# lucidrains/audiolm-pytorch

Hardware: NVIDIA H100
Metric: CoarseTransformer tokens/sec fwd+bwd seq2048 (higher is better)
Workload: dtype bf16

## Files before the change

audiolm_pytorch_b200/csrc/attn_bwd_wgmma.cu:

```cuda
#include "alm_common.cuh"
#include "ptx_sm90.cuh"

namespace alm {

constexpr int AB_T = 128;
constexpr int AB_THREADS = 256;
constexpr int AB_STAGES = 3;
template <int D>
struct AttBwdCfg {
  static constexpr int TQ = D == 128 ? 64 : 128;
  static constexpr int ROW_BYTES = SwizzledTile<D>::ROW_BYTES;
  static constexpr int KV_HALF = AB_T * ROW_BYTES, KV_TILE = AB_T * D * 2;
  static constexpr int Q_HALF = TQ * ROW_BYTES, Q_TILE = TQ * D * 2;
  static constexpr int DS_HALF = AB_T * 128, DS_TILE = AB_T * TQ * 2;
  static constexpr int DQ_STAGE = D == 128 ? 2 * 64 * 64 * 4 : 0;
  static constexpr int SMEM = 2 * KV_TILE + 2 * AB_STAGES * Q_TILE + 2 * DS_TILE + DQ_STAGE + AB_STAGES * 2 * TQ * 4 + 256;
};
constexpr float LOG2E = 1.4426950408889634f;

struct AttnBwdParams {
  const float* lse;
  const float* delta;
  const uint32_t* kmask;
  int kb_stride;
  const float* bias;
  float* dbias;
  long long bias_hs, bias_rs;
  float* dq_acc;
  __nv_bfloat16* dk;
  __nv_bfloat16* dv;
  long long lddk, lddv;
  int b, h, n_q, n_k, n_q_pad;
  int causal;
  float scale, scale_log2;
};

__device__ __forceinline__ float ex2_approx(float x) {
  float y;
  asm("ex2.approx.ftz.f32 %0, %1;" : "=f"(y) : "f"(x));
  return y;
}

template <int KS>
__device__ __forceinline__ void pack_a_frags(const float (&v)[8 * KS], uint32_t (&a)[KS][4]) {
#pragma unroll
  for (int kk = 0; kk < KS; ++kk) {
    a[kk][0] = pack_bf16x2(v[8 * kk + 0], v[8 * kk + 1]);
    a[kk][1] = pack_bf16x2(v[8 * kk + 2], v[8 * kk + 3]);
    a[kk][2] = pack_bf16x2(v[8 * kk + 4], v[8 * kk + 5]);
    a[kk][3] = pack_bf16x2(v[8 * kk + 6], v[8 * kk + 7]);
  }
}

template <int D>
__device__ __forceinline__ void store_acc(const float (&acc)[D / 2], __nv_bfloat16* row0, __nv_bfloat16* row1, int c_lane) {
#pragma unroll
  for (int h = 0; h < 2; ++h) {
    __nv_bfloat16* dst = h == 0 ? row0 : row1;
    if (dst == nullptr) continue;
#pragma unroll
    for (int g = 0; g < D / 8; ++g)
      *reinterpret_cast<uint32_t*>(dst + 8 * g + c_lane) = pack_bf16x2(acc[4 * g + 2 * h], acc[4 * g + 2 * h + 1]);
  }
}

template <int TQ>
__device__ __forceinline__ uint64_t attn_bwd_keep_bits(const DropoutArgs& d, uint32_t qrow0, uint32_t key0) {
  uint64_t bits = 0;
#pragma unroll
  for (int cc = 0; cc < TQ / 16; ++cc) {
    const uint32_t i0 = qrow0 + 16 * cc;
    const uint4 dr = dropout_draw(d, i0, key0);
#pragma unroll
    for (int gh = 0; gh < 2; ++gh)
#pragma unroll
      for (int h = 0; h < 2; ++h)
#pragma unroll
        for (int c = 0; c < 2; ++c)
          if (dropout_pick(d, dr, i0 + 8 * gh + c, key0 + 8 * h)) bits |= 1ull << (8 * cc + 4 * gh + 2 * h + c);
  }
  return bits;
}

constexpr uint32_t AB_DS_BAR = 1;
constexpr uint32_t AB_WG_BAR = 2;

constexpr int AB_TRACE_ITERS = 128, AB_TRACE_STAMPS = 8;
#ifdef ALM_ATTN_BWD_TRACE
__device__ long long g_attn_bwd_trace[2][AB_TRACE_ITERS][AB_TRACE_STAMPS];
#define AB_STAMP(i)                                                                                   \
  do {                                                                                                \
    if (blockIdx.x == 0 && (threadIdx.x & 127) == 0 && it < AB_TRACE_ITERS)                           \
      g_attn_bwd_trace[threadIdx.x >> 7][it][i] = clock64();                                          \
  } while (0)
#else
#define AB_STAMP(i)
#endif

template <int AB_D, bool HAS_BIAS, bool DROPOUT>
__global__ void __launch_bounds__(AB_THREADS, 1)
mqa_attn_bwd_kernel(const __grid_constant__ CUtensorMap tmQ, const __grid_constant__ CUtensorMap tmK,
                    const __grid_constant__ CUtensorMap tmV, const __grid_constant__ CUtensorMap tmdO,
                    const __grid_constant__ CUtensorMap tmdQ, const AttnBwdParams p, const DropoutArgs drop) {
  extern __shared__ __align__(1024) uint8_t smem[];
  if ((smem_u32(smem) & 1023u) != 0) __trap();
  using Tile = SwizzledTile<AB_D>;
  using Cfg = AttBwdCfg<AB_D>;
  constexpr int TQ = Cfg::TQ, AB_TILE = Cfg::Q_TILE, AB_DS_TILE = Cfg::DS_TILE;
  constexpr int KV_HALF = Cfg::KV_HALF, Q_HALF = Cfg::Q_HALF, DS_HALF = Cfg::DS_HALF;
  constexpr int WG_ROWS = 64 * Cfg::ROW_BYTES;
  uint8_t* sK = smem;
  uint8_t* sV = sK + Cfg::KV_TILE;
  uint8_t* sQ = sV + Cfg::KV_TILE;
  uint8_t* sdO = sQ + AB_STAGES * AB_TILE;
  uint8_t* sDS = sdO + AB_STAGES * AB_TILE;
  uint8_t* sDQ = sDS + 2 * AB_DS_TILE;
  float* sLse = reinterpret_cast<float*>(sDQ + Cfg::DQ_STAGE);
  float* sDelta = sLse + AB_STAGES * TQ;
  uint64_t* bars = reinterpret_cast<uint64_t*>(sDelta + AB_STAGES * TQ);
  uint64_t* kv_full = bars;
  uint64_t* qdo_full = bars + 1;
  uint64_t* qdo_empty = qdo_full + AB_STAGES;

  const int warp = threadIdx.x >> 5, lane = threadIdx.x & 31;
  const int kb = blockIdx.x / p.b, batch = blockIdx.x % p.b;
  const int k0 = kb * AB_T;
  const int off = p.n_k - p.n_q;
  const int n_qblocks = (p.n_q + TQ - 1) / TQ;
  int qb_min = 0;
  if (p.causal && k0 - off > 0) qb_min = (k0 - off) / TQ;
  const int q_per_head = n_qblocks - qb_min;
  const int n_iter = q_per_head > 0 ? q_per_head * p.h : 0;

  if (threadIdx.x == 0) {
    tma_prefetch_desc(&tmQ); tma_prefetch_desc(&tmK); tma_prefetch_desc(&tmV); tma_prefetch_desc(&tmdO);
    tma_prefetch_desc(&tmdQ);
    mbar_init(kv_full, 1);
    for (int i = 0; i < AB_STAGES; ++i) { mbar_init(&qdo_full[i], 1); mbar_init(&qdo_empty[i], 8); }
    fence_mbar_init();
  }
  __syncthreads();

  auto issue_qdo = [&](int it) {
    const int st = it % AB_STAGES;
    const int head = it / q_per_head, qb = qb_min + it % q_per_head;
    const size_t roff = ((size_t)batch * p.h + head) * p.n_q_pad + (size_t)qb * TQ;
    if (elect_one_sync()) {
      mbar_arrive_expect_tx(&qdo_full[st], 2 * AB_TILE + 2 * TQ * 4);
#pragma unroll
      for (int hf = 0; hf < Tile::HALVES; ++hf) {
        tma_load_3d(sQ + st * AB_TILE + hf * Q_HALF, &tmQ, &qdo_full[st], head * AB_D + hf * Tile::HW, qb * TQ, batch);
        tma_load_3d(sdO + st * AB_TILE + hf * Q_HALF, &tmdO, &qdo_full[st], head * AB_D + hf * Tile::HW, qb * TQ, batch);
      }
      bulk_copy_g2s(sLse + st * TQ, p.lse + roff, TQ * 4, &qdo_full[st]);
      bulk_copy_g2s(sDelta + st * TQ, p.delta + roff, TQ * 4, &qdo_full[st]);
    }
    __syncwarp();
  };
  if (warp == 0 && n_iter > 0) {
    if (elect_one_sync()) {
      mbar_arrive_expect_tx(kv_full, 2 * Cfg::KV_TILE);
#pragma unroll
      for (int hf = 0; hf < Tile::HALVES; ++hf) {
        tma_load_3d(sK + hf * KV_HALF, &tmK, kv_full, hf * Tile::HW, k0, batch);
        tma_load_3d(sV + hf * KV_HALF, &tmV, kv_full, hf * Tile::HW, k0, batch);
      }
    }
    __syncwarp();
    for (int it = 0; it < min(n_iter, AB_STAGES); ++it) issue_qdo(it);
  }

  const int cw = warp >> 2;
  const int wl = warp & 3;
  const int r_base = cw * 64 + wl * 16 + (lane >> 2);
  const int c_lane = 2 * (lane & 3);
  int kj[2];
  bool key_ok[2];
#pragma unroll
  for (int h = 0; h < 2; ++h) {
    kj[h] = k0 + r_base + 8 * h;
    key_ok[h] = kj[h] < p.n_k;
    if (key_ok[h] && p.kmask != nullptr)
      key_ok[h] = (p.kmask[(size_t)batch * p.kb_stride + (kj[h] >> 5)] >> (kj[h] & 31)) & 1u;
  }
  float dv[AB_D / 2], dk[AB_D / 2];
#pragma unroll
  for (int e = 0; e < AB_D / 2; ++e) { dv[e] = 0.f; dk[e] = 0.f; }
  const uint32_t k_all = smem_u32(sK);
  const uint32_t k_addr = k_all + cw * WG_ROWS, v_addr = smem_u32(sV) + cw * WG_ROWS;
  const bool wg_leader = (threadIdx.x & 127) == 0;
  if (n_iter > 0) mbar_wait(kv_full, 0);
  int stage = 0;
  uint32_t phase = 0;
  for (int it = 0; it < n_iter; ++it) {
    const int head = it / q_per_head;
    const int q0 = (qb_min + it % q_per_head) * TQ;
    [[maybe_unused]] const long long bias_head = HAS_BIAS ? (long long)head * p.bias_hs : 0;
    AB_STAMP(0);
    mbar_wait(&qdo_full[stage], phase);
    AB_STAMP(1);
    const uint32_t q_addr = smem_u32(sQ + stage * AB_TILE), do_addr = smem_u32(sdO + stage * AB_TILE);
    const uint32_t ds_addr = smem_u32(sDS + (it & 1) * AB_DS_TILE);
    float st[TQ / 2], dpt[TQ / 2];
    wgmma_fence();
#pragma unroll
    for (int k = 0; k < AB_D / 16; ++k)
      wgmma_ss<TQ>(st, Tile::kmajor(k_addr, k, KV_HALF), Tile::kmajor(q_addr, k, Q_HALF), k > 0 ? 1u : 0u);
    wgmma_commit();
#pragma unroll
    for (int k = 0; k < AB_D / 16; ++k)
      wgmma_ss<TQ>(dpt, Tile::kmajor(v_addr, k, KV_HALF), Tile::kmajor(do_addr, k, Q_HALF), k > 0 ? 1u : 0u);
    wgmma_commit();
    AB_STAMP(2);
    [[maybe_unused]] uint64_t keep = 0;
    if constexpr (DROPOUT)
      keep = attn_bwd_keep_bits<TQ>(drop, ((uint32_t)batch * p.h + head) * (uint32_t)p.n_q_pad + q0 + c_lane, kj[0]);
    const float* lse_s = sLse + stage * TQ;
    const float* del_s = sDelta + stage * TQ;
    const bool tile_full = (q0 + TQ <= p.n_q) && (!p.causal || k0 + AB_T - 1 <= q0 + off);
    const int q_end = tile_full ? INT_MAX : p.n_q;
    int q_lo[2];
#pragma unroll
    for (int h = 0; h < 2; ++h) q_lo[h] = tile_full || !p.causal ? INT_MIN : kj[h] - off;
    auto visible = [&](int h, int qi) { return key_ok[h] & (qi >= q_lo[h]) & (qi < q_end); };
    auto bias_index = [&](int h, int qi) {
      return bias_head + (long long)min(qi, p.n_q - 1) * p.bias_rs + min(kj[h], p.n_k - 1);
    };
    wgmma_wait<1>();
    wgmma_fence_acc(st);
#pragma unroll
    for (int g = 0; g < TQ / 8; ++g)
#pragma unroll
      for (int c = 0; c < 2; ++c) {
        const int col = 8 * g + c_lane + c;
        const int qi = q0 + col;
        const float lv = lse_s[col];
#pragma unroll
        for (int h = 0; h < 2; ++h) {
          const int e = 4 * g + 2 * h + c;
          float shift = -lv;
          if constexpr (HAS_BIAS) shift = fmaf(__ldg(p.bias + bias_index(h, qi)), LOG2E, shift);
          const float x = fmaf(st[e], p.scale_log2, shift);
          st[e] = ex2_approx(visible(h, qi) ? x : -INFINITY);
        }
      }
    AB_STAMP(3);
    uint32_t pa[TQ / 16][4];
    if constexpr (DROPOUT) {
      float pz[TQ / 2];
#pragma unroll
      for (int e = 0; e < TQ / 2; ++e) pz[e] = ((keep >> e) & 1u) ? st[e] * drop.scale : 0.f;
      pack_a_frags(pz, pa);
    } else {
      pack_a_frags(st, pa);
    }
    wgmma_fence_acc(dv);
    wgmma_fence();
#pragma unroll
    for (int kk = 0; kk < TQ / 16; ++kk)
      wgmma_rs<AB_D, 1>(dv, pa[kk], Tile::mnmajor(do_addr, kk, Q_HALF), 1u);
    wgmma_commit();
    wgmma_wait<1>();
    wgmma_fence_acc(dpt);
    if (it > 0) {
      if (wg_leader) bulk_wait_group_read<0>();
      named_bar_sync(AB_WG_BAR + cw, 128);
    }
#pragma unroll
    for (int g = 0; g < TQ / 8; ++g) {
#pragma unroll
      for (int c = 0; c < 2; ++c) {
        const int col = 8 * g + c_lane + c;
        const int qi = q0 + col;
        const float dl = del_s[col];
#pragma unroll
        for (int h = 0; h < 2; ++h) {
          const int e = 4 * g + 2 * h + c;
          const bool ok = visible(h, qi);
          float ds;
          if constexpr (DROPOUT)
            ds = ok ? st[e] * ((((keep >> e) & 1u) ? dpt[e] * drop.scale : 0.f) - dl) : 0.f;
          else
            ds = ok ? st[e] * (dpt[e] - dl) : 0.f;
          if constexpr (HAS_BIAS) {
            if (ok && p.dbias != nullptr) atomicAdd(p.dbias + bias_index(h, qi), ds);
          }
          dpt[e] = ds * p.scale;
        }
      }
#pragma unroll
      for (int h = 0; h < 2; ++h) {
        const int row = r_base + 8 * h;
        const uint32_t a = ds_addr + (g >> 3) * DS_HALF + row * 128 + (((g & 7) ^ (row & 7)) << 4) + 2 * c_lane;
        st_shared_u32(a, pack_bf16x2(dpt[4 * g + 2 * h], dpt[4 * g + 2 * h + 1]));
      }
    }
    AB_STAMP(4);
    fence_proxy_async_smem();
    named_bar_sync(AB_DS_BAR, 2 * 128);
    AB_STAMP(5);
    if (warp == 0 && it >= 1 && it - 1 + AB_STAGES < n_iter) {
      const int prev = stage == 0 ? AB_STAGES - 1 : stage - 1;
      mbar_wait(&qdo_empty[prev], stage == 0 ? phase ^ 1u : phase);
      issue_qdo(it - 1 + AB_STAGES);
    }
    constexpr int DQ_N = AB_D == 128 ? 64 : AB_D;
    float dq[DQ_N / 2];
    wgmma_fence_acc(dk);
    wgmma_fence();
#pragma unroll
    for (int kk = 0; kk < TQ / 16; ++kk)
      wgmma_ss<AB_D, 0, 1>(dk, wgmma_desc_sw128(ds_addr + (kk >> 2) * DS_HALF + cw * 8192 + (kk & 3) * 32, 1024, 16),
                           Tile::mnmajor(q_addr, kk, Q_HALF), 1u);
    const uint32_t dq_a = ds_addr + (AB_D == 128 ? 0 : cw * DS_HALF);
    const uint32_t dq_b = k_all + (AB_D == 128 ? cw * KV_HALF : 0);
#pragma unroll
    for (int kk = 0; kk < AB_T / 16; ++kk)
      wgmma_ss<DQ_N, 1, 1>(dq, wgmma_desc_sw128(dq_a + kk * 2048, 1024, 8192), Tile::mnmajor(dq_b, kk, KV_HALF),
                           kk > 0 ? 1u : 0u);
    wgmma_commit();
    wgmma_wait<0>();
    wgmma_fence_acc(dv);
    wgmma_fence_acc(dk);
    wgmma_fence_acc(dq);
    AB_STAMP(6);
    if (lane == 0) mbar_arrive(&qdo_empty[stage]);
    const uint32_t stg = AB_D == 128 ? smem_u32(sDQ) + cw * (Cfg::DQ_STAGE / 2)
                                     : smem_u32(sDS + ((it + 1) & 1) * AB_DS_TILE) + cw * 8192;
    constexpr uint32_t BOX_STRIDE = AB_D == 128 ? 8192 : DS_HALF;
#pragma unroll
    for (int h = 0; h < 2; ++h) {
      const int row = wl * 16 + (lane >> 2) + 8 * h;
#pragma unroll
      for (int g = 0; g < DQ_N / 8; ++g) {
        const int byte = 32 * (g & 3) + 4 * c_lane;
        st_shared_f32x2(stg + (g >> 2) * BOX_STRIDE + row * 128 + ((((byte >> 4) ^ (row & 7)) << 4) | (byte & 15)),
                        dq[4 * g + 2 * h], dq[4 * g + 2 * h + 1]);
      }
    }
    fence_proxy_async_smem();
    named_bar_sync(AB_WG_BAR + cw, 128);
    if (wg_leader) {
      const int dq_col = head * AB_D + (AB_D == 128 ? cw * 64 : 0), dq_row = q0 + (AB_D == 128 ? 0 : cw * 64);
      tma_reduce_add_3d(&tmdQ, stg, dq_col, dq_row, batch);
      if constexpr (DQ_N == 64) tma_reduce_add_3d(&tmdQ, stg + BOX_STRIDE, dq_col + 32, dq_row, batch);
      bulk_commit_group();
    }
    AB_STAMP(7);
    if (++stage == AB_STAGES) { stage = 0; phase ^= 1u; }
  }
  if (wg_leader) bulk_wait_group<0>();
  __nv_bfloat16* rv[2];
  __nv_bfloat16* rk[2];
#pragma unroll
  for (int h = 0; h < 2; ++h) {
    const bool in = kj[h] < p.n_k;
    rv[h] = in ? p.dv + ((size_t)batch * p.n_k + kj[h]) * p.lddv : nullptr;
    rk[h] = in ? p.dk + ((size_t)batch * p.n_k + kj[h]) * p.lddk : nullptr;
  }
  store_acc<AB_D>(dv, rv[0], rv[1], c_lane);
  store_acc<AB_D>(dk, rk[0], rk[1], c_lane);
}

__global__ void attn_dq_convert_kernel(const float4* __restrict__ acc, __nv_bfloat16* __restrict__ dq, long long lddq,
                                       long long rows, int cols4) {
  const long long i = (long long)blockIdx.x * blockDim.x + threadIdx.x;
  if (i >= rows * cols4) return;
  const long long r = i / cols4;
  const int c = (int)(i - r * cols4);
  const float4 v = acc[i];
  *reinterpret_cast<uint2*>(dq + r * lddq + 4 * c) = make_uint2(pack_bf16x2(v.x, v.y), pack_bf16x2(v.z, v.w));
}

}

namespace alm {
template <int D>
static int attn_bwd_launch(const void* q, int64_t ldq, const void* k, int64_t ldk, int64_t k_bstride, const void* v,
                           int64_t ldv, int64_t v_bstride, const void* d_o, int64_t lddo, void* dq, int64_t lddq,
                           const AttnBwdParams& p, const DropoutArgs& dargs, cudaStream_t stream) {
  using Tile = SwizzledTile<D>;
  using Cfg = AttBwdCfg<D>;
  const int b = p.b, h = p.h, n_q = p.n_q, n_k = p.n_k;
  CUtensorMap tmQ, tmK, tmV, tmdO;
  {
    uint64_t dims[3] = {(uint64_t)h * D, (uint64_t)n_q, (uint64_t)b};
    uint64_t strides[3] = {2, (uint64_t)ldq * 2, (uint64_t)n_q * ldq * 2};
    uint32_t box[3] = {Tile::HW, Cfg::TQ, 1};
    int rc = make_tensor_map(&tmQ, q, 2, 3, dims, strides, box, Tile::SWIZZLE);
    if (rc != ALM_OK) return rc;
    strides[1] = (uint64_t)lddo * 2;
    strides[2] = (uint64_t)n_q * lddo * 2;
    rc = make_tensor_map(&tmdO, d_o, 2, 3, dims, strides, box, Tile::SWIZZLE);
    if (rc != ALM_OK) return rc;
  }
  {
    uint64_t dims[3] = {(uint64_t)D, (uint64_t)n_k, (uint64_t)b};
    uint64_t strides[3] = {2, (uint64_t)ldk * 2, (uint64_t)k_bstride * 2};
    uint32_t box[3] = {Tile::HW, AB_T, 1};
    int rc = make_tensor_map(&tmK, k, 2, 3, dims, strides, box, Tile::SWIZZLE);
    if (rc != ALM_OK) return rc;
    strides[1] = (uint64_t)ldv * 2;
    strides[2] = (uint64_t)v_bstride * 2;
    rc = make_tensor_map(&tmV, v, 2, 3, dims, strides, box, Tile::SWIZZLE);
    if (rc != ALM_OK) return rc;
  }
  CUtensorMap tmdQ;
  {
    uint64_t dims[3] = {(uint64_t)h * D, (uint64_t)n_q, (uint64_t)b};
    uint64_t strides[3] = {4, (uint64_t)h * D * 4, (uint64_t)n_q * h * D * 4};
    uint32_t box[3] = {32, 64, 1};
    int rc = make_tensor_map(&tmdQ, p.dq_acc, 4, 3, dims, strides, box, 128);
    if (rc != ALM_OK) return rc;
  }
  static bool attr_set = false;
  if (!attr_set) {
    ALM_CUDA_OK(cudaFuncSetAttribute(mqa_attn_bwd_kernel<D, false, false>, cudaFuncAttributeMaxDynamicSharedMemorySize, Cfg::SMEM));
    ALM_CUDA_OK(cudaFuncSetAttribute(mqa_attn_bwd_kernel<D, true, false>, cudaFuncAttributeMaxDynamicSharedMemorySize, Cfg::SMEM));
    ALM_CUDA_OK(cudaFuncSetAttribute(mqa_attn_bwd_kernel<D, false, true>, cudaFuncAttributeMaxDynamicSharedMemorySize, Cfg::SMEM));
    ALM_CUDA_OK(cudaFuncSetAttribute(mqa_attn_bwd_kernel<D, true, true>, cudaFuncAttributeMaxDynamicSharedMemorySize, Cfg::SMEM));
    attr_set = true;
  }
  dim3 grid(((n_k + AB_T - 1) / AB_T) * b);
  const bool drop = dargs.thr < 65536u;
  if (p.bias != nullptr && drop)
    mqa_attn_bwd_kernel<D, true, true><<<grid, AB_THREADS, Cfg::SMEM, stream>>>(tmQ, tmK, tmV, tmdO, tmdQ, p, dargs);
  else if (p.bias != nullptr)
    mqa_attn_bwd_kernel<D, true, false><<<grid, AB_THREADS, Cfg::SMEM, stream>>>(tmQ, tmK, tmV, tmdO, tmdQ, p, dargs);
  else if (drop)
    mqa_attn_bwd_kernel<D, false, true><<<grid, AB_THREADS, Cfg::SMEM, stream>>>(tmQ, tmK, tmV, tmdO, tmdQ, p, dargs);
  else
    mqa_attn_bwd_kernel<D, false, false><<<grid, AB_THREADS, Cfg::SMEM, stream>>>(tmQ, tmK, tmV, tmdO, tmdQ, p, dargs);
  ALM_CHECK_LAUNCH();
  const long long rows = (long long)b * n_q;
  const int cols4 = h * D / 4;
  attn_dq_convert_kernel<<<(unsigned)ceil_div(rows * cols4, 256LL), 256, 0, stream>>>(
      reinterpret_cast<const float4*>(p.dq_acc), (__nv_bfloat16*)dq, lddq, rows, cols4);
  ALM_CHECK_LAUNCH();
  ALM_LAUNCHED(2);
  return ALM_OK;
}
}

extern "C" int alm_mqa_attn_bwd_dh(const void* q, int64_t ldq, const void* k, int64_t ldk, int64_t k_bstride,
                                   const void* v, int64_t ldv, int64_t v_bstride, const void* d_o, int64_t lddo,
                                   const void* key_mask, const float* lse, const float* delta, int n_q_pad, void* dq,
                                   int64_t lddq, float* dq_acc, void* dk, int64_t lddk, void* dv, int64_t lddv,
                                   const float* bias, float* dbias, int64_t bias_hstride, int64_t bias_rstride, int b,
                                   int h, int n_q, int n_k, int causal, float scale, float dropout_p, uint64_t seed,
                                   uint32_t site, int dim_head, alm_stream_t stream_) {
  using namespace alm;
  cudaStream_t stream = reinterpret_cast<cudaStream_t>(stream_);
  ALM_REQUIRE(dim_head == 32 || dim_head == 64 || dim_head == 128, ALM_ERR_UNSUPPORTED);
  ALM_REQUIRE(q && k && v && d_o && lse && delta && dq && dq_acc && dk && dv, ALM_ERR_ARG);
  ALM_REQUIRE(b > 0 && h > 0 && n_q > 0 && n_k >= n_q, ALM_ERR_ARG);
  ALM_REQUIRE(n_q_pad % AB_T == 0 && n_q_pad >= n_q, ALM_ERR_ARG);
  ALM_REQUIRE(dropout_p >= 0.f && dropout_p < 1.f, ALM_ERR_ARG);
  ALM_REQUIRE(dropout_p == 0.f || n_q_pad == (n_q + AB_T - 1) / AB_T * AB_T, ALM_ERR_ARG);
  ALM_REQUIRE((long long)b * h * n_q_pad < (1ll << 32), ALM_ERR_UNSUPPORTED);
  if (bias != nullptr) {
    ALM_REQUIRE(bias_rstride >= n_k && bias_rstride % 4 == 0 && bias_hstride % 4 == 0, ALM_ERR_ALIGN);
    ALM_REQUIRE((reinterpret_cast<uintptr_t>(bias) & 15u) == 0, ALM_ERR_ALIGN);
  } else {
    ALM_REQUIRE(dbias == nullptr, ALM_ERR_ARG);
  }
  ALM_REQUIRE(ldq % 8 == 0 && ldk % 8 == 0 && ldv % 8 == 0 && lddo % 8 == 0 && lddq % 8 == 0 && lddk % 8 == 0 &&
                  lddv % 8 == 0 && k_bstride % 8 == 0 && v_bstride % 8 == 0,
              ALM_ERR_ALIGN);
  AttnBwdParams p;
  p.lse = lse; p.delta = delta;
  p.kmask = reinterpret_cast<const uint32_t*>(key_mask);
  p.kb_stride = (n_k + 127) / 128 * 4;
  p.dq_acc = dq_acc; p.dk = (__nv_bfloat16*)dk; p.dv = (__nv_bfloat16*)dv;
  p.lddk = lddk; p.lddv = lddv;
  p.bias = bias; p.dbias = dbias; p.bias_hs = bias_hstride; p.bias_rs = bias_rstride;
  p.b = b; p.h = h; p.n_q = n_q; p.n_k = n_k; p.n_q_pad = n_q_pad;
  p.causal = causal;
  p.scale = scale;
  p.scale_log2 = scale * LOG2E;
  const DropoutArgs dargs = make_dropout_args(dropout_p, seed, site);
#define ALM_ATT_BWD(DD) \
  attn_bwd_launch<DD>(q, ldq, k, ldk, k_bstride, v, ldv, v_bstride, d_o, lddo, dq, lddq, p, dargs, stream)
  if (dim_head == 32) return ALM_ATT_BWD(32);
  if (dim_head == 64) return ALM_ATT_BWD(64);
  return ALM_ATT_BWD(128);
#undef ALM_ATT_BWD
}

extern "C" int alm_mqa_attn_bwd(const void* q, int64_t ldq, const void* k, int64_t ldk, int64_t k_bstride,
                                const void* v, int64_t ldv, int64_t v_bstride, const void* d_o, int64_t lddo,
                                const void* key_mask, const float* lse, const float* delta, int n_q_pad, void* dq,
                                int64_t lddq, float* dq_acc, void* dk, int64_t lddk, void* dv, int64_t lddv, const float* bias,
                                float* dbias, int64_t bias_hstride, int64_t bias_rstride, int b, int h, int n_q,
                                int n_k, int causal, float scale, float dropout_p, uint64_t seed, uint32_t site,
                                alm_stream_t stream_) {
  return alm_mqa_attn_bwd_dh(q, ldq, k, ldk, k_bstride, v, ldv, v_bstride, d_o, lddo, key_mask, lse, delta, n_q_pad, dq,
                             lddq, dq_acc, dk, lddk, dv, lddv, bias, dbias, bias_hstride, bias_rstride, b, h, n_q, n_k,
                             causal, scale, dropout_p, seed, site, 64, stream_);
}

#ifdef ALM_ATTN_BWD_TRACE
extern "C" int alm_attn_bwd_trace_read(long long* dst) {
  ALM_CUDA_OK(cudaMemcpyFromSymbol(dst, alm::g_attn_bwd_trace, sizeof(alm::g_attn_bwd_trace)));
  return ALM_OK;
}
#endif
```

audiolm_pytorch_b200/csrc/attn_fwd_wgmma.cu:

```cuda
#include "alm_common.cuh"
#include "ptx_sm90.cuh"

namespace alm {

constexpr int ATT_BM = 128;
constexpr int ATT_BN = 128;
constexpr int ATT_THREADS = 384;
template <int D>
struct AttFwdCfg {
  static constexpr int KV_STAGES = D == 128 ? 3 : 4;
  static constexpr int HALF_BYTES = 128 * SwizzledTile<D>::ROW_BYTES;
  static constexpr int TILE_BYTES = 128 * D * 2;
  static constexpr int SMEM_BYTES = TILE_BYTES * (1 + 2 * KV_STAGES) + 256;
};

struct AttnFwdParams {
  __nv_bfloat16* o;
  float* lse;
  const uint32_t* kmask;
  int kb_stride;
  const float* bias;
  long long bias_hs, bias_rs;
  long long ldo, lse_stride;
  int b, h, n_q, n_k;
  int causal;
  float scale_log2;
  int n_q_pad;
  uint32_t drop_row0;
  DropoutArgs drop;
};

__device__ __forceinline__ float att_ex2(float x) {
  float y;
  asm("ex2.approx.ftz.f32 %0, %1;" : "=f"(y) : "f"(x));
  return y;
}

__device__ __forceinline__ uint64_t attn_fwd_keep_bits(const DropoutArgs& d, uint32_t qrow, uint32_t kbase, int c_lane) {
  const uint32_t odd = qrow & 1u;
  uint64_t bits = 0;
#pragma unroll
  for (int kk = 0; kk < ATT_BN / 16; ++kk) {
    const uint32_t j0 = kbase + 16 * kk + c_lane;
    const uint4 own = dropout_draw(d, qrow, j0 + odd);
    const uint32_t ra = __shfl_xor_sync(0xffffffffu, odd ? own.x : own.y, 4);
    const uint32_t rb = __shfl_xor_sync(0xffffffffu, odd ? own.z : own.w, 4);
    const uint4 other = odd ? make_uint4(0u, ra, 0u, rb) : make_uint4(ra, 0u, rb, 0u);
#pragma unroll
    for (int c = 0; c < 2; ++c) {
      const uint4 dr = (uint32_t)c == odd ? own : other;
#pragma unroll
      for (int half = 0; half < 2; ++half)
#pragma unroll
        for (int h = 0; h < 2; ++h)
          if (dropout_pick(d, dr, qrow + 8 * h, j0 + 8 * half + c)) bits |= 1ull << (8 * kk + 4 * half + 2 * h + c);
    }
  }
  return bits;
}

template <int ATT_D, bool HAS_BIAS, bool DROPOUT>
__global__ void __launch_bounds__(ATT_THREADS, 1)
mqa_attn_fwd_kernel(const __grid_constant__ CUtensorMap tmQ, const __grid_constant__ CUtensorMap tmK,
                    const __grid_constant__ CUtensorMap tmV, const AttnFwdParams p) {
  using Tile = SwizzledTile<ATT_D>;
  using Cfg = AttFwdCfg<ATT_D>;
  constexpr int ATT_KV_STAGES = Cfg::KV_STAGES, ATT_TILE_BYTES = Cfg::TILE_BYTES, HALF = Cfg::HALF_BYTES;
  constexpr bool REG_HANDOFF = ATT_D == 128;
  extern __shared__ __align__(1024) uint8_t smem_raw[];
  uint8_t* smem = smem_raw;
  if ((smem_u32(smem) & 1023u) != 0) __trap();
  uint8_t* sQ = smem;
  uint8_t* sK = sQ + ATT_TILE_BYTES;
  uint8_t* sV = sK + ATT_KV_STAGES * ATT_TILE_BYTES;
  uint64_t* bars = reinterpret_cast<uint64_t*>(sV + ATT_KV_STAGES * ATT_TILE_BYTES);
  uint64_t* q_full = bars;
  uint64_t* kv_full = bars + 1;
  uint64_t* kv_empty = kv_full + ATT_KV_STAGES;

  const int warp = threadIdx.x >> 5;
  const int lane = threadIdx.x & 31;
  const int wg = warp >> 2;
  const int n_qblocks = (p.n_q + ATT_BM - 1) / ATT_BM;
  const int qb = n_qblocks - 1 - (int)blockIdx.x;
  const int head = blockIdx.y;
  const int batch = blockIdx.z;
  const int q0 = qb * ATT_BM;
  const int off = p.n_k - p.n_q;
  int kv_end = p.n_k;
  if (p.causal) kv_end = min(p.n_k, q0 + ATT_BM + off);
  const int n_tiles = kv_end > 0 ? (kv_end + ATT_BN - 1) / ATT_BN : 0;

  if (threadIdx.x == 0) {
    tma_prefetch_desc(&tmQ);
    tma_prefetch_desc(&tmK);
    tma_prefetch_desc(&tmV);
    mbar_init(q_full, 1);
    for (int i = 0; i < ATT_KV_STAGES; ++i) {
      mbar_init(&kv_full[i], 1);
      mbar_init(&kv_empty[i], 8);
    }
    fence_mbar_init();
  }
  __syncthreads();

  if (wg == 0) {
    if constexpr (REG_HANDOFF) setmaxnreg_dec<40>();
    if (warp == 0 && n_tiles > 0) {
      if (elect_one_sync()) {
        mbar_arrive_expect_tx(q_full, ATT_TILE_BYTES);
#pragma unroll
        for (int hf = 0; hf < Tile::HALVES; ++hf)
          tma_load_3d(sQ + hf * HALF, &tmQ, q_full, head * ATT_D + hf * Tile::HW, q0, batch);
      }
      __syncwarp();
      int stage = 0;
      uint32_t phase = 0;
      for (int j = 0; j < n_tiles; ++j) {
        mbar_wait(&kv_empty[stage], phase ^ 1u);
        if (elect_one_sync()) {
          mbar_arrive_expect_tx(&kv_full[stage], 2 * ATT_TILE_BYTES);
#pragma unroll
          for (int hf = 0; hf < Tile::HALVES; ++hf) {
            tma_load_3d(sK + stage * ATT_TILE_BYTES + hf * HALF, &tmK, &kv_full[stage], hf * Tile::HW, j * ATT_BN, batch);
            tma_load_3d(sV + stage * ATT_TILE_BYTES + hf * HALF, &tmV, &kv_full[stage], hf * Tile::HW, j * ATT_BN, batch);
          }
        }
        __syncwarp();
        if (++stage == ATT_KV_STAGES) { stage = 0; phase ^= 1u; }
      }
    }
    return;
  }

  if constexpr (REG_HANDOFF) setmaxnreg_inc<232>();
  const int cw = wg - 1;
  const int r_base = cw * 64 + (warp & 3) * 16 + (lane >> 2);
  const int c_lane = 2 * (lane & 3);
  constexpr float kLog2e = 1.4426950408889634f;
  float m_run[2] = {-INFINITY, -INFINITY}, l_run[2] = {0.f, 0.f};
  float o_acc[ATT_D / 2];
#pragma unroll
  for (int d = 0; d < ATT_D / 2; ++d) o_acc[d] = 0.f;
  int q_limit[2];
  [[maybe_unused]] const float* brow[2];
#pragma unroll
  for (int h = 0; h < 2; ++h) {
    const int qi = q0 + r_base + 8 * h;
    q_limit[h] = min(p.causal ? qi + off : p.n_k - 1, p.n_k - 1);
    if constexpr (HAS_BIAS) brow[h] = p.bias + (long long)head * p.bias_hs + (long long)min(qi, p.n_q - 1) * p.bias_rs;
  }
  const uint32_t* mrow = p.kmask ? p.kmask + (long long)batch * p.kb_stride : nullptr;
  const uint32_t q_addr = smem_u32(sQ) + cw * 64 * Tile::ROW_BYTES;
  [[maybe_unused]] const uint32_t drop_row =
      p.drop_row0 + ((uint32_t)batch * p.h + head) * (uint32_t)p.n_q_pad + q0 + r_base;

  if (n_tiles > 0) mbar_wait(q_full, 0);
  int stage = 0;
  uint32_t phase = 0;
  for (int j = 0; j < n_tiles; ++j) {
    mbar_wait(&kv_full[stage], phase);
    const uint32_t k_addr = smem_u32(sK + stage * ATT_TILE_BYTES);
    const uint32_t v_addr = smem_u32(sV + stage * ATT_TILE_BYTES);
    float s[ATT_BN / 2];
    wgmma_fence();
#pragma unroll
    for (int k = 0; k < ATT_D / 16; ++k)
      wgmma_ss<ATT_BN>(s, Tile::kmajor(q_addr, k, HALF), Tile::kmajor(k_addr, k, HALF), k > 0 ? 1u : 0u);
    wgmma_commit();
    [[maybe_unused]] uint64_t keep = 0;
    if constexpr (DROPOUT) keep = attn_fwd_keep_bits(p.drop, drop_row, j * ATT_BN, c_lane);
    wgmma_wait<0>();
    wgmma_fence_acc(s);

    const int kbase = j * ATT_BN;
    const bool tile_full = mrow == nullptr && kbase + ATT_BN <= p.n_k && (!p.causal || kbase + ATT_BN - 1 <= q0 + off);
    uint32_t valid[4] = {0xFFFFFFFFu, 0xFFFFFFFFu, 0xFFFFFFFFu, 0xFFFFFFFFu};
    if (!tile_full && mrow != nullptr) {
      const uint4 mv = __ldg(reinterpret_cast<const uint4*>(mrow + j * 4));
      valid[0] = mv.x; valid[1] = mv.y; valid[2] = mv.z; valid[3] = mv.w;
    }
    uint32_t pa[ATT_BN / 16][4];
#pragma unroll
    for (int h = 0; h < 2; ++h) {
#pragma unroll
      for (int g = 0; g < ATT_BN / 8; ++g)
#pragma unroll
        for (int c = 0; c < 2; ++c) {
          const int col = 8 * g + c_lane + c;
          float v = s[4 * g + 2 * h + c] * p.scale_log2;
          if constexpr (HAS_BIAS) {
            if (kbase + col < p.bias_rs) v = fmaf(__ldg(brow[h] + kbase + col), kLog2e, v);
          }
          if (!tile_full) {
            const bool ok = kbase + col <= q_limit[h] && ((valid[col >> 5] >> (col & 31)) & 1u);
            if (!ok) v = -INFINITY;
          }
          s[4 * g + 2 * h + c] = v;
        }
      float m_tile = -INFINITY;
#pragma unroll
      for (int g = 0; g < ATT_BN / 8; ++g) m_tile = fmaxf(m_tile, fmaxf(s[4 * g + 2 * h], s[4 * g + 2 * h + 1]));
      m_tile = fmaxf(m_tile, __shfl_xor_sync(0xffffffffu, m_tile, 1));
      m_tile = fmaxf(m_tile, __shfl_xor_sync(0xffffffffu, m_tile, 2));
      const float m_new = fmaxf(m_run[h], m_tile);
      const float m_use = (m_new == -INFINITY) ? 0.f : m_new;
      const float alpha = att_ex2(m_run[h] - m_use);
      float l_tile = 0.f;
#pragma unroll
      for (int g = 0; g < ATT_BN / 8; ++g)
#pragma unroll
        for (int c = 0; c < 2; ++c) {
          const float pv = att_ex2(s[4 * g + 2 * h + c] - m_use);
          s[4 * g + 2 * h + c] = pv;
          l_tile += pv;
        }
      l_run[h] = fmaf(l_run[h], alpha, l_tile);
      m_run[h] = m_new;
#pragma unroll
      for (int g = 0; g < ATT_D / 8; ++g) {
        o_acc[4 * g + 2 * h] *= alpha;
        o_acc[4 * g + 2 * h + 1] *= alpha;
      }
    }
    if constexpr (DROPOUT) {
#pragma unroll
      for (int e = 0; e < ATT_BN / 2; ++e) s[e] = ((keep >> e) & 1u) ? s[e] * p.drop.scale : 0.f;
    }
#pragma unroll
    for (int kk = 0; kk < ATT_BN / 16; ++kk) {
      pa[kk][0] = pack_bf16x2(s[8 * kk + 0], s[8 * kk + 1]);
      pa[kk][1] = pack_bf16x2(s[8 * kk + 2], s[8 * kk + 3]);
      pa[kk][2] = pack_bf16x2(s[8 * kk + 4], s[8 * kk + 5]);
      pa[kk][3] = pack_bf16x2(s[8 * kk + 6], s[8 * kk + 7]);
    }
    wgmma_fence_acc(o_acc);
    wgmma_fence();
#pragma unroll
    for (int kk = 0; kk < ATT_BN / 16; ++kk)
      wgmma_rs<ATT_D, 1>(o_acc, pa[kk], Tile::mnmajor(v_addr, kk, HALF), 1u);
    wgmma_commit();
    wgmma_wait<0>();
    wgmma_fence_acc(o_acc);
    if (lane == 0) mbar_arrive(&kv_empty[stage]);
    if (++stage == ATT_KV_STAGES) { stage = 0; phase ^= 1u; }
  }

#pragma unroll
  for (int h = 0; h < 2; ++h) {
    float l_tot = l_run[h];
    l_tot += __shfl_xor_sync(0xffffffffu, l_tot, 1);
    l_tot += __shfl_xor_sync(0xffffffffu, l_tot, 2);
    const int qi = q0 + r_base + 8 * h;
    if (qi < p.n_q) {
      const float inv = l_tot > 0.f ? 1.f / l_tot : 0.f;
      __nv_bfloat16* dst = p.o + ((long long)batch * p.n_q + qi) * p.ldo + head * ATT_D + c_lane;
#pragma unroll
      for (int g = 0; g < ATT_D / 8; ++g)
        *reinterpret_cast<uint32_t*>(dst + 8 * g) = pack_bf16x2(o_acc[4 * g + 2 * h] * inv, o_acc[4 * g + 2 * h + 1] * inv);
      if (p.lse != nullptr && (lane & 3) == 0) {
        const float lse = l_tot > 0.f ? (m_run[h] + log2f(l_tot)) : INFINITY;
        p.lse[((long long)batch * p.h + head) * p.lse_stride + qi] = lse;
      }
    }
  }
}

}

namespace alm {
__global__ void pack_key_mask_kernel(const uint8_t* __restrict__ mask, uint32_t* __restrict__ bits, int n_k, int words,
                                     long long total) {
  const long long i = (long long)blockIdx.x * (blockDim.x >> 5) + (threadIdx.x >> 5);
  if (i >= total) return;
  const long long b = i / words;
  const int k = (int)(i - b * words) * 32 + (threadIdx.x & 31);
  const bool on = k < n_k && mask[b * n_k + k] != 0;
  const uint32_t v = __ballot_sync(0xffffffffu, on);
  if ((threadIdx.x & 31) == 0) bits[i] = v;
}
}

extern "C" int alm_pack_key_mask(const void* key_mask, void* bits, int b, int n_k, alm_stream_t stream_) {
  using namespace alm;
  cudaStream_t stream = reinterpret_cast<cudaStream_t>(stream_);
  ALM_REQUIRE(key_mask && bits && b > 0 && n_k > 0, ALM_ERR_ARG);
  const int words = (n_k + 127) / 128 * 4;
  const long long total = (long long)b * words;
  const long long blocks = ceil_div(total, 8LL);
  ALM_REQUIRE(blocks <= INT_MAX, ALM_ERR_UNSUPPORTED);
  pack_key_mask_kernel<<<(unsigned)blocks, 256, 0, stream>>>(reinterpret_cast<const uint8_t*>(key_mask),
                                                            reinterpret_cast<uint32_t*>(bits), n_k, words, total);
  ALM_CHECK_LAUNCH();
  ALM_LAUNCHED(1);
  return ALM_OK;
}

namespace alm {
template <int D>
static int attn_fwd_launch(const void* q, int64_t ldq, const void* k, int64_t ldk, int64_t k_bstride, const void* v,
                           int64_t ldv, int64_t v_bstride, const void* key_mask, void* o, int64_t ldo, float* lse,
                           const float* bias, int b, bool drop, AttnFwdParams p, cudaStream_t stream) {
  using Tile = SwizzledTile<D>;
  constexpr int SMEM = AttFwdCfg<D>::SMEM_BYTES;
  const int h = p.h, n_q = p.n_q, n_k = p.n_k;
  static bool attr_set = false;
  if (!attr_set) {
    ALM_CUDA_OK(cudaFuncSetAttribute(mqa_attn_fwd_kernel<D, false, false>, cudaFuncAttributeMaxDynamicSharedMemorySize, SMEM));
    ALM_CUDA_OK(cudaFuncSetAttribute(mqa_attn_fwd_kernel<D, true, false>, cudaFuncAttributeMaxDynamicSharedMemorySize, SMEM));
    ALM_CUDA_OK(cudaFuncSetAttribute(mqa_attn_fwd_kernel<D, false, true>, cudaFuncAttributeMaxDynamicSharedMemorySize, SMEM));
    ALM_CUDA_OK(cudaFuncSetAttribute(mqa_attn_fwd_kernel<D, true, true>, cudaFuncAttributeMaxDynamicSharedMemorySize, SMEM));
    attr_set = true;
  }
  constexpr int kMaxGridZ = 65535;
  const int n_launch = ceil_div(b, kMaxGridZ);
  for (int b0 = 0; b0 < b; b0 += kMaxGridZ) {
    const int nb = min(b - b0, kMaxGridZ);
    CUtensorMap tmQ, tmK, tmV;
    {
      uint64_t dims[3] = {(uint64_t)h * D, (uint64_t)n_q, (uint64_t)nb};
      uint64_t strides[3] = {2, (uint64_t)ldq * 2, (uint64_t)n_q * ldq * 2};
      uint32_t box[3] = {Tile::HW, ATT_BM, 1};
      int rc = make_tensor_map(&tmQ, reinterpret_cast<const __nv_bfloat16*>(q) + (long long)b0 * n_q * ldq, 2, 3, dims,
                               strides, box, Tile::SWIZZLE);
      if (rc != ALM_OK) return rc;
    }
    {
      uint64_t dims[3] = {(uint64_t)D, (uint64_t)n_k, (uint64_t)nb};
      uint64_t strides[3] = {2, (uint64_t)ldk * 2, (uint64_t)k_bstride * 2};
      uint32_t box[3] = {Tile::HW, ATT_BN, 1};
      int rc = make_tensor_map(&tmK, reinterpret_cast<const __nv_bfloat16*>(k) + (long long)b0 * k_bstride, 2, 3, dims,
                               strides, box, Tile::SWIZZLE);
      if (rc != ALM_OK) return rc;
      strides[1] = (uint64_t)ldv * 2;
      strides[2] = (uint64_t)v_bstride * 2;
      rc = make_tensor_map(&tmV, reinterpret_cast<const __nv_bfloat16*>(v) + (long long)b0 * v_bstride, 2, 3, dims,
                           strides, box, Tile::SWIZZLE);
      if (rc != ALM_OK) return rc;
    }
    p.o = reinterpret_cast<__nv_bfloat16*>(o) + (long long)b0 * n_q * ldo;
    p.lse = lse != nullptr ? lse + (long long)b0 * h * p.lse_stride : nullptr;
    p.kmask = key_mask != nullptr ? reinterpret_cast<const uint32_t*>(key_mask) + (long long)b0 * p.kb_stride : nullptr;
    p.b = nb;
    p.drop_row0 = (uint32_t)((long long)b0 * h * p.n_q_pad);
    const dim3 grid((n_q + ATT_BM - 1) / ATT_BM, h, nb);
    if (bias != nullptr && drop)
      mqa_attn_fwd_kernel<D, true, true><<<grid, ATT_THREADS, SMEM, stream>>>(tmQ, tmK, tmV, p);
    else if (bias != nullptr)
      mqa_attn_fwd_kernel<D, true, false><<<grid, ATT_THREADS, SMEM, stream>>>(tmQ, tmK, tmV, p);
    else if (drop)
      mqa_attn_fwd_kernel<D, false, true><<<grid, ATT_THREADS, SMEM, stream>>>(tmQ, tmK, tmV, p);
    else
      mqa_attn_fwd_kernel<D, false, false><<<grid, ATT_THREADS, SMEM, stream>>>(tmQ, tmK, tmV, p);
    ALM_CHECK_LAUNCH();
  }
  ALM_LAUNCHED(n_launch);
  return ALM_OK;
}
}

extern "C" int alm_mqa_attn_fwd_dh(const void* q, int64_t ldq, const void* k, int64_t ldk, int64_t k_bstride,
                                   const void* v, int64_t ldv, int64_t v_bstride, const void* key_mask, void* o,
                                   int64_t ldo, float* lse, int64_t lse_stride, const float* bias,
                                   int64_t bias_hstride, int64_t bias_rstride, int b, int h, int n_q, int n_k,
                                   int causal, float scale, float dropout_p, uint64_t seed, uint32_t site,
                                   int dim_head, alm_stream_t stream_) {
  using namespace alm;
  cudaStream_t stream = reinterpret_cast<cudaStream_t>(stream_);
  ALM_REQUIRE(dim_head == 32 || dim_head == 64 || dim_head == 128, ALM_ERR_UNSUPPORTED);
  ALM_REQUIRE(q && k && v && o, ALM_ERR_ARG);
  ALM_REQUIRE(b > 0 && h > 0 && n_q > 0 && n_k > 0 && n_k >= n_q, ALM_ERR_ARG);
  ALM_REQUIRE(dropout_p >= 0.f && dropout_p < 1.f, ALM_ERR_ARG);
  ALM_REQUIRE((long long)b * h * ((n_q + 127) / 128 * 128) < (1ll << 32), ALM_ERR_UNSUPPORTED);
  ALM_REQUIRE(ldq % 8 == 0 && ldk % 8 == 0 && ldv % 8 == 0 && ldo % 8 == 0, ALM_ERR_ALIGN);
  ALM_REQUIRE(k_bstride % 8 == 0 && v_bstride % 8 == 0, ALM_ERR_ALIGN);
  ALM_REQUIRE((reinterpret_cast<uintptr_t>(o) & 15u) == 0, ALM_ERR_ALIGN);
  if (bias != nullptr) {
    ALM_REQUIRE(bias_rstride >= n_k && bias_rstride % 4 == 0 && bias_hstride % 4 == 0, ALM_ERR_ALIGN);
    ALM_REQUIRE((reinterpret_cast<uintptr_t>(bias) & 15u) == 0, ALM_ERR_ALIGN);
  }

  AttnFwdParams p;
  p.kb_stride = (n_k + 127) / 128 * 4;
  p.bias = bias;
  p.bias_hs = bias_hstride;
  p.bias_rs = bias_rstride;
  p.ldo = ldo;
  p.lse_stride = lse_stride;
  p.h = h; p.n_q = n_q; p.n_k = n_k;
  p.causal = causal;
  p.scale_log2 = scale * 1.4426950408889634f;
  p.n_q_pad = (n_q + 127) / 128 * 128;
  p.drop = make_dropout_args(dropout_p, seed, site);
  const bool drop = dropout_p > 0.f;
#define ALM_ATT_FWD(DD) \
  attn_fwd_launch<DD>(q, ldq, k, ldk, k_bstride, v, ldv, v_bstride, key_mask, o, ldo, lse, bias, b, drop, p, stream)
  if (dim_head == 32) return ALM_ATT_FWD(32);
  if (dim_head == 64) return ALM_ATT_FWD(64);
  return ALM_ATT_FWD(128);
#undef ALM_ATT_FWD
}

extern "C" int alm_mqa_attn_fwd(const void* q, int64_t ldq, const void* k, int64_t ldk, int64_t k_bstride,
                                const void* v, int64_t ldv, int64_t v_bstride, const void* key_mask, void* o,
                                int64_t ldo, float* lse, int64_t lse_stride, const float* bias, int64_t bias_hstride,
                                int64_t bias_rstride, int b, int h, int n_q, int n_k, int causal, float scale,
                                float dropout_p, uint64_t seed, uint32_t site, alm_stream_t stream_) {
  return alm_mqa_attn_fwd_dh(q, ldq, k, ldk, k_bstride, v, ldv, v_bstride, key_mask, o, ldo, lse, lse_stride, bias,
                             bias_hstride, bias_rstride, b, h, n_q, n_k, causal, scale, dropout_p, seed, site, 64,
                             stream_);
}
```

Before: 753,800.

## Specialize attention masking per warp and defer softmax scale multiplies

```diff
diff --git a/audiolm_pytorch_b200/csrc/attn_bwd_wgmma.cu b/audiolm_pytorch_b200/csrc/attn_bwd_wgmma.cu
--- a/audiolm_pytorch_b200/csrc/attn_bwd_wgmma.cu
+++ b/audiolm_pytorch_b200/csrc/attn_bwd_wgmma.cu
@@ -35,6 +35,11 @@
   float scale, scale_log2;
 };
 
+template <bool E>
+struct AbEdge {
+  static constexpr bool value = E;
+};
+
 __device__ __forceinline__ float ex2_approx(float x) {
   float y;
   asm("ex2.approx.ftz.f32 %0, %1;" : "=f"(y) : "f"(x));
@@ -53,14 +58,16 @@
 }
 
 template <int D>
-__device__ __forceinline__ void store_acc(const float (&acc)[D / 2], __nv_bfloat16* row0, __nv_bfloat16* row1, int c_lane) {
+__device__ __forceinline__ void store_acc(const float (&acc)[D / 2], float mul, __nv_bfloat16* row0,
+                                          __nv_bfloat16* row1, int c_lane) {
 #pragma unroll
   for (int h = 0; h < 2; ++h) {
     __nv_bfloat16* dst = h == 0 ? row0 : row1;
     if (dst == nullptr) continue;
 #pragma unroll
     for (int g = 0; g < D / 8; ++g)
-      *reinterpret_cast<uint32_t*>(dst + 8 * g + c_lane) = pack_bf16x2(acc[4 * g + 2 * h], acc[4 * g + 2 * h + 1]);
+      *reinterpret_cast<uint32_t*>(dst + 8 * g + c_lane) =
+          pack_bf16x2(acc[4 * g + 2 * h] * mul, acc[4 * g + 2 * h + 1] * mul);
   }
 }
 
@@ -183,6 +190,7 @@
     if (key_ok[h] && p.kmask != nullptr)
       key_ok[h] = (p.kmask[(size_t)batch * p.kb_stride + (kj[h] >> 5)] >> (kj[h] & 31)) & 1u;
   }
+  const int warp_key_last = k0 + cw * 64 + wl * 16 + 15;
   float dv[AB_D / 2], dk[AB_D / 2];
 #pragma unroll
   for (int e = 0; e < AB_D / 2; ++e) { dv[e] = 0.f; dk[e] = 0.f; }
@@ -217,33 +225,40 @@
       keep = attn_bwd_keep_bits<TQ>(drop, ((uint32_t)batch * p.h + head) * (uint32_t)p.n_q_pad + q0 + c_lane, kj[0]);
     const float* lse_s = sLse + stage * TQ;
     const float* del_s = sDelta + stage * TQ;
-    const bool tile_full = (q0 + TQ <= p.n_q) && (!p.causal || k0 + AB_T - 1 <= q0 + off);
-    const int q_end = tile_full ? INT_MAX : p.n_q;
+    const bool interior = (q0 + TQ <= p.n_q) && (!p.causal || warp_key_last - off <= q0);
+    const int q_end = p.n_q;
     int q_lo[2];
 #pragma unroll
-    for (int h = 0; h < 2; ++h) q_lo[h] = tile_full || !p.causal ? INT_MIN : kj[h] - off;
+    for (int h = 0; h < 2; ++h) q_lo[h] = p.causal ? kj[h] - off : INT_MIN;
     auto visible = [&](int h, int qi) { return key_ok[h] & (qi >= q_lo[h]) & (qi < q_end); };
     auto bias_index = [&](int h, int qi) {
       return bias_head + (long long)min(qi, p.n_q - 1) * p.bias_rs + min(kj[h], p.n_k - 1);
     };
     wgmma_wait<1>();
     wgmma_fence_acc(st);
-#pragma unroll
-    for (int g = 0; g < TQ / 8; ++g)
-#pragma unroll
-      for (int c = 0; c < 2; ++c) {
-        const int col = 8 * g + c_lane + c;
-        const int qi = q0 + col;
-        const float lv = lse_s[col];
-#pragma unroll
-        for (int h = 0; h < 2; ++h) {
-          const int e = 4 * g + 2 * h + c;
-          float shift = -lv;
-          if constexpr (HAS_BIAS) shift = fmaf(__ldg(p.bias + bias_index(h, qi)), LOG2E, shift);
-          const float x = fmaf(st[e], p.scale_log2, shift);
-          st[e] = ex2_approx(visible(h, qi) ? x : -INFINITY);
+    auto exponentials = [&](auto edge_c) {
+      constexpr bool EDGE = decltype(edge_c)::value;
+#pragma unroll
+      for (int g = 0; g < TQ / 8; ++g)
+#pragma unroll
+        for (int c = 0; c < 2; ++c) {
+          const int col = 8 * g + c_lane + c;
+          const int qi = q0 + col;
+          const float lv = lse_s[col];
+#pragma unroll
+          for (int h = 0; h < 2; ++h) {
+            const int e = 4 * g + 2 * h + c;
+            float shift = -lv;
+            if constexpr (HAS_BIAS) shift = fmaf(__ldg(p.bias + bias_index(h, qi)), LOG2E, shift);
+            const float x = fmaf(st[e], p.scale_log2, shift);
+            st[e] = ex2_approx((EDGE ? visible(h, qi) : key_ok[h]) ? x : -INFINITY);
+          }
         }
-      }
+    };
+    if (interior)
+      exponentials(AbEdge<false>{});
+    else
+      exponentials(AbEdge<true>{});
     AB_STAMP(3);
     uint32_t pa[TQ / 16][4];
     if constexpr (DROPOUT) {
@@ -266,35 +281,43 @@
       if (wg_leader) bulk_wait_group_read<0>();
       named_bar_sync(AB_WG_BAR + cw, 128);
     }
-#pragma unroll
-    for (int g = 0; g < TQ / 8; ++g) {
-#pragma unroll
-      for (int c = 0; c < 2; ++c) {
-        const int col = 8 * g + c_lane + c;
-        const int qi = q0 + col;
-        const float dl = del_s[col];
+    auto ds_tile = [&](auto edge_c) {
+      constexpr bool EDGE = decltype(edge_c)::value;
+#pragma unroll
+      for (int g = 0; g < TQ / 8; ++g) {
+#pragma unroll
+        for (int c = 0; c < 2; ++c) {
+          const int col = 8 * g + c_lane + c;
+          const int qi = q0 + col;
+          const float dl = del_s[col];
+#pragma unroll
+          for (int h = 0; h < 2; ++h) {
+            const int e = 4 * g + 2 * h + c;
+            const bool ok = EDGE ? visible(h, qi) : key_ok[h];
+            float ds;
+            if constexpr (DROPOUT)
+              ds = st[e] * ((((keep >> e) & 1u) ? dpt[e] * drop.scale : 0.f) - dl);
+            else
+              ds = st[e] * (dpt[e] - dl);
+            if constexpr (EDGE) ds = ok ? ds : 0.f;
+            if constexpr (HAS_BIAS) {
+              if (ok && p.dbias != nullptr) atomicAdd(p.dbias + bias_index(h, qi), ds);
+            }
+            dpt[e] = ds;
+          }
+        }
 #pragma unroll
         for (int h = 0; h < 2; ++h) {
-          const int e = 4 * g + 2 * h + c;
-          const bool ok = visible(h, qi);
-          float ds;
-          if constexpr (DROPOUT)
-            ds = ok ? st[e] * ((((keep >> e) & 1u) ? dpt[e] * drop.scale : 0.f) - dl) : 0.f;
-          else
-            ds = ok ? st[e] * (dpt[e] - dl) : 0.f;
-          if constexpr (HAS_BIAS) {
-            if (ok && p.dbias != nullptr) atomicAdd(p.dbias + bias_index(h, qi), ds);
-          }
-          dpt[e] = ds * p.scale;
+          const int row = r_base + 8 * h;
+          const uint32_t a = ds_addr + (g >> 3) * DS_HALF + row * 128 + (((g & 7) ^ (row & 7)) << 4) + 2 * c_lane;
+          st_shared_u32(a, pack_bf16x2(dpt[4 * g + 2 * h], dpt[4 * g + 2 * h + 1]));
         }
       }
-#pragma unroll
-      for (int h = 0; h < 2; ++h) {
-        const int row = r_base + 8 * h;
-        const uint32_t a = ds_addr + (g >> 3) * DS_HALF + row * 128 + (((g & 7) ^ (row & 7)) << 4) + 2 * c_lane;
-        st_shared_u32(a, pack_bf16x2(dpt[4 * g + 2 * h], dpt[4 * g + 2 * h + 1]));
-      }
-    }
+    };
+    if (interior)
+      ds_tile(AbEdge<false>{});
+    else
+      ds_tile(AbEdge<true>{});
     AB_STAMP(4);
     fence_proxy_async_smem();
     named_bar_sync(AB_DS_BAR, 2 * 128);
@@ -358,17 +381,18 @@
     rv[h] = in ? p.dv + ((size_t)batch * p.n_k + kj[h]) * p.lddv : nullptr;
     rk[h] = in ? p.dk + ((size_t)batch * p.n_k + kj[h]) * p.lddk : nullptr;
   }
-  store_acc<AB_D>(dv, rv[0], rv[1], c_lane);
-  store_acc<AB_D>(dk, rk[0], rk[1], c_lane);
+  store_acc<AB_D>(dv, 1.f, rv[0], rv[1], c_lane);
+  store_acc<AB_D>(dk, p.scale, rk[0], rk[1], c_lane);
 }
 
 __global__ void attn_dq_convert_kernel(const float4* __restrict__ acc, __nv_bfloat16* __restrict__ dq, long long lddq,
-                                       long long rows, int cols4) {
+                                       long long rows, int cols4, float scale) {
   const long long i = (long long)blockIdx.x * blockDim.x + threadIdx.x;
   if (i >= rows * cols4) return;
   const long long r = i / cols4;
   const int c = (int)(i - r * cols4);
-  const float4 v = acc[i];
+  float4 v = acc[i];
+  v.x *= scale; v.y *= scale; v.z *= scale; v.w *= scale;
   *reinterpret_cast<uint2*>(dq + r * lddq + 4 * c) = make_uint2(pack_bf16x2(v.x, v.y), pack_bf16x2(v.z, v.w));
 }
 
@@ -435,7 +459,7 @@
   const long long rows = (long long)b * n_q;
   const int cols4 = h * D / 4;
   attn_dq_convert_kernel<<<(unsigned)ceil_div(rows * cols4, 256LL), 256, 0, stream>>>(
-      reinterpret_cast<const float4*>(p.dq_acc), (__nv_bfloat16*)dq, lddq, rows, cols4);
+      reinterpret_cast<const float4*>(p.dq_acc), (__nv_bfloat16*)dq, lddq, rows, cols4, p.scale);
   ALM_CHECK_LAUNCH();
   ALM_LAUNCHED(2);
   return ALM_OK;
diff --git a/audiolm_pytorch_b200/csrc/attn_fwd_wgmma.cu b/audiolm_pytorch_b200/csrc/attn_fwd_wgmma.cu
--- a/audiolm_pytorch_b200/csrc/attn_fwd_wgmma.cu
+++ b/audiolm_pytorch_b200/csrc/attn_fwd_wgmma.cu
@@ -28,6 +28,11 @@
   int n_q_pad;
   uint32_t drop_row0;
   DropoutArgs drop;
+};
+
+template <bool EDGE_>
+struct AttTileClass {
+  static constexpr bool EDGE = EDGE_;
 };
 
 __device__ __forceinline__ float att_ex2(float x) {
@@ -150,6 +155,7 @@
     q_limit[h] = min(p.causal ? qi + off : p.n_k - 1, p.n_k - 1);
     if constexpr (HAS_BIAS) brow[h] = p.bias + (long long)head * p.bias_hs + (long long)min(qi, p.n_q - 1) * p.bias_rs;
   }
+  const int warp_limit = min(p.causal ? q0 + cw * 64 + (warp & 3) * 16 + off : p.n_k - 1, p.n_k - 1);
   const uint32_t* mrow = p.kmask ? p.kmask + (long long)batch * p.kb_stride : nullptr;
   const uint32_t q_addr = smem_u32(sQ) + cw * 64 * Tile::ROW_BYTES;
   [[maybe_unused]] const uint32_t drop_row =
@@ -174,30 +180,47 @@
     wgmma_fence_acc(s);
 
     const int kbase = j * ATT_BN;
-    const bool tile_full = mrow == nullptr && kbase + ATT_BN <= p.n_k && (!p.causal || kbase + ATT_BN - 1 <= q0 + off);
-    uint32_t valid[4] = {0xFFFFFFFFu, 0xFFFFFFFFu, 0xFFFFFFFFu, 0xFFFFFFFFu};
-    if (!tile_full && mrow != nullptr) {
-      const uint4 mv = __ldg(reinterpret_cast<const uint4*>(mrow + j * 4));
-      valid[0] = mv.x; valid[1] = mv.y; valid[2] = mv.z; valid[3] = mv.w;
-    }
-    uint32_t pa[ATT_BN / 16][4];
+    uint4 mv = make_uint4(0xFFFFFFFFu, 0xFFFFFFFFu, 0xFFFFFFFFu, 0xFFFFFFFFu);
+    if (mrow != nullptr) mv = __ldg(reinterpret_cast<const uint4*>(mrow + j * 4));
+
+    if constexpr (HAS_BIAS) {
+#pragma unroll
+      for (int h = 0; h < 2; ++h)
+#pragma unroll
+        for (int g = 0; g < ATT_BN / 8; ++g)
+#pragma unroll
+          for (int c = 0; c < 2; ++c) {
+            const int col = 8 * g + c_lane + c;
+            float v = s[4 * g + 2 * h + c] * p.scale_log2;
+            if (kbase + col < p.bias_rs) v = fmaf(__ldg(brow[h] + kbase + col), kLog2e, v);
+            s[4 * g + 2 * h + c] = v;
+          }
+    }
+    const bool all_keys = (mv.x & mv.y & mv.z & mv.w) == 0xFFFFFFFFu;
+    const uint32_t kw[4] = {mv.x >> c_lane, mv.y >> c_lane, mv.z >> c_lane, mv.w >> c_lane};
+    auto hide_invisible = [&](auto cls) {
+      constexpr bool EDGE = decltype(cls)::EDGE;
+      [[maybe_unused]] const int lim[2] = {q_limit[0] - kbase - c_lane, q_limit[1] - kbase - c_lane};
+#pragma unroll
+      for (int g = 0; g < ATT_BN / 8; ++g)
+#pragma unroll
+        for (int c = 0; c < 2; ++c) {
+          const bool key_on = (kw[g >> 2] >> (8 * (g & 3) + c)) & 1u;
+#pragma unroll
+          for (int h = 0; h < 2; ++h) {
+            bool ok = key_on;
+            if constexpr (EDGE) ok = ok && 8 * g + c <= lim[h];
+            if (!ok) s[4 * g + 2 * h + c] = -INFINITY;
+          }
+        }
+    };
+    if (HAS_BIAS || kbase + ATT_BN - 1 > warp_limit)
+      hide_invisible(AttTileClass<true>{});
+    else if (!all_keys)
+      hide_invisible(AttTileClass<false>{});
+    constexpr bool kRaw = !HAS_BIAS;
 #pragma unroll
     for (int h = 0; h < 2; ++h) {
-#pragma unroll
-      for (int g = 0; g < ATT_BN / 8; ++g)
-#pragma unroll
-        for (int c = 0; c < 2; ++c) {
-          const int col = 8 * g + c_lane + c;
-          float v = s[4 * g + 2 * h + c] * p.scale_log2;
-          if constexpr (HAS_BIAS) {
-            if (kbase + col < p.bias_rs) v = fmaf(__ldg(brow[h] + kbase + col), kLog2e, v);
-          }
-          if (!tile_full) {
-            const bool ok = kbase + col <= q_limit[h] && ((valid[col >> 5] >> (col & 31)) & 1u);
-            if (!ok) v = -INFINITY;
-          }
-          s[4 * g + 2 * h + c] = v;
-        }
       float m_tile = -INFINITY;
 #pragma unroll
       for (int g = 0; g < ATT_BN / 8; ++g) m_tile = fmaxf(m_tile, fmaxf(s[4 * g + 2 * h], s[4 * g + 2 * h + 1]));
@@ -205,13 +228,15 @@
       m_tile = fmaxf(m_tile, __shfl_xor_sync(0xffffffffu, m_tile, 2));
       const float m_new = fmaxf(m_run[h], m_tile);
       const float m_use = (m_new == -INFINITY) ? 0.f : m_new;
-      const float alpha = att_ex2(m_run[h] - m_use);
+      const float sc = kRaw ? p.scale_log2 : 1.f;
+      const float alpha = att_ex2((m_run[h] - m_use) * sc);
+      const float m_shift = -m_use * sc;
       float l_tile = 0.f;
 #pragma unroll
       for (int g = 0; g < ATT_BN / 8; ++g)
 #pragma unroll
         for (int c = 0; c < 2; ++c) {
-          const float pv = att_ex2(s[4 * g + 2 * h + c] - m_use);
+          const float pv = att_ex2(fmaf(s[4 * g + 2 * h + c], sc, m_shift));
           s[4 * g + 2 * h + c] = pv;
           l_tile += pv;
         }
@@ -223,6 +248,7 @@
         o_acc[4 * g + 2 * h + 1] *= alpha;
       }
     }
+    uint32_t pa[ATT_BN / 16][4];
     if constexpr (DROPOUT) {
 #pragma unroll
       for (int e = 0; e < ATT_BN / 2; ++e) s[e] = ((keep >> e) & 1u) ? s[e] * p.drop.scale : 0.f;
@@ -259,7 +285,8 @@
       for (int g = 0; g < ATT_D / 8; ++g)
         *reinterpret_cast<uint32_t*>(dst + 8 * g) = pack_bf16x2(o_acc[4 * g + 2 * h] * inv, o_acc[4 * g + 2 * h + 1] * inv);
       if (p.lse != nullptr && (lane & 3) == 0) {
-        const float lse = l_tot > 0.f ? (m_run[h] + log2f(l_tot)) : INFINITY;
+        const float m_log2 = HAS_BIAS ? m_run[h] : m_run[h] * p.scale_log2;
+        const float lse = l_tot > 0.f ? (m_log2 + log2f(l_tot)) : INFINITY;
         p.lse[((long long)batch * p.h + head) * p.lse_stride + qi] = lse;
       }
     }
```

New measurement: 764,100 (median of 6 runs). 1.01x the previous value.
